# SLebailly/Ignis-MasterThesis

Measured on AMD Instinct MI355X. Metric: Mrays/s (primary+secondary) at fixed spp; per-pixel L2 vs CPU ref, higher is better.
Workload: dtype f32; 1 GPU; diamond_scene.json 1000x1000, 256 spp = 32 iterations x spi 8, path tracer max_depth 64, seed 0; scene=diamond_scene.json, width=1000, height=1000, spp=256, spi=8, parallelism=single GPU

## Files before the change

### ignis-masterthesis_amd/csrc/igx_device.hip

```cpp
#include "igx.h"

#include "device_math.h"
#include "device_scene.h"
#include "igx_kernels.h"
#include "../host/bvh_build.h"
#include "../host/light_select.h"
#include "../host/lds_plan.h"
#include "../host/aov_plan.h"
#include "../host/film_tools.h"

#include <hip/hip_runtime.h>

#include <algorithm>
#include <array>
#include <chrono>
#include <map>
#include <cmath>
#include <cstring>
#include <condition_variable>
#include <deque>
#include <memory>
#include <mutex>
#include <string>
#include <thread>
// ... 32 lines not shown

constexpr int NSH = 64;
constexpr int CSTRIDE = 16;
constexpr int CROW = NSH * CSTRIDE;
constexpr int WAVES_PER_BLOCK = BLOCK / 64;
#ifndef EXTEND_TREELET
#define EXTEND_TREELET 1
#endif
#ifndef SHADOW_TREELET
#define SHADOW_TREELET 1
#endif
#ifndef IGX_CLAIM_NEXT
#define IGX_CLAIM_NEXT 1
#endif
#ifndef IGX_LIVE_GRID
#define IGX_LIVE_GRID 1
#endif
[[maybe_unused]] constexpr int GRID_QUANTUM = NSH / WAVES_PER_BLOCK;

struct PathBuf {
    float4* p0;
    float4* p1;
    float4* p2;
    float2* p3;
    int shard_cap;
    int c_base;
};
struct ShadowBuf {
    float4* s0;
    float4* s1;
    float4* s2;
    int shard_cap;
    float4* aov_nee;
};
struct HitBuf {
    float4* h;
    int* prim;
};

#ifndef IGX_AOV
#define IGX_AOV 1
#endif
struct FrameArgs {
    int width, height, spi, iter, frame, seed;
    int tile_size, tile_offset, tile_stride, tiles_x;
    int num_rays;
    const float* rays;
    int chunk_pixel0;
    int chunk_pixels;
    int chunk_iters;
    float inv_spi;
    int gen_n;
    int classify;
    int dynamic;
    int shadow_classes;
    int reverse;
    int probe_sample;
    float4* aov_di;
    float4* aov_nee;
};

__device__ __forceinline__ void slot_coords(const FrameArgs& fa, int slot, int& lp, int& sample, int& iter) {
    const int per_iter = fa.chunk_pixels * fa.spi;
    const int it = slot / per_iter;
    const int r = slot - it * per_iter;
    const int q = r / fa.spi;
    lp = fa.chunk_pixel0 + q;
    sample = r - q * fa.spi;
    iter = fa.iter + it;
}

#ifndef IGX_PIXEL_BLOCKS
#define IGX_PIXEL_BLOCKS 1
#endif
__device__ __forceinline__ void block_order(int r, int w, int& x, int& y) {
    const int pair = r / (2 * w), q = r - pair * 2 * w;
    x = (q >> 3) * 4 + (q & 3);
    y = 2 * pair + ((q >> 2) & 1);
}
template <bool BLOCKED = true>
__device__ __forceinline__ bool local_to_global(const FrameArgs& fa, int lp, int& x, int& y) {
    if (fa.num_rays > 0) { x = lp; y = 0; return lp < fa.num_rays; }
    if (fa.tile_size <= 0) {
        if (BLOCKED && IGX_PIXEL_BLOCKS && (fa.width & 3) == 0 && (fa.height & 1) == 0) block_order(lp, fa.width, x, y);
        else { y = lp / fa.width; x = lp - y * fa.width; }
        return true;
    }
    int T = fa.tile_size;
// ... 390 lines not shown
}

__device__ __forceinline__ void phase_mark(TraceStats& st, unsigned long long& last, int k) {
    __builtin_amdgcn_s_waitcnt(0);
    __builtin_amdgcn_sched_barrier(0);
    const unsigned long long now = __builtin_amdgcn_s_memtime();
    __builtin_amdgcn_sched_barrier(0);
    st.cyc[k] += now - last;
    last = now;
}
template <bool STATS, int V>
__device__ __forceinline__ bool extend_step(const FrameArgs& fa, const SceneView& sv, const TStack& ts, PathState& ps, f3& Lacc,
                                            bool& has_l, bool& has_shadow, ShadowRec& sr, TraceStats& st) {
    float tmin, tmax;
    uint32_t rflags;
    ray_extent(fa, sv, ps.depth, ps.slot, tmin, tmax, rflags);
    int hit_ent, hit_prim;
    float hu = 0, hv = 0;
    trace_path_ray<STATS, V>(sv, ps.inside, ps.o, ps.d, tmin, tmax, rflags, ts, hit_ent, hit_prim, hu, hv, st);
    if (STATS && hit_ent >= 0) st.hits++;
    return shade_step<variant_full(V)>(fa, sv, ps, hit_ent, hit_prim, tmax, hu, hv, Lacc, has_l, has_shadow, sr);
}

__device__ __forceinline__ void add_radiance(float4* L, int slot, f3 c) {
    float4 l = L[slot];
    L[slot] = make_float4(l.x + c.x, l.y + c.y, l.z + c.z, 0);
}
template <bool ON = true>
__device__ __forceinline__ void add_aov(float4* A, int slot, f3 c) {
    if (ON && IGX_AOV && A) add_radiance(A, slot, c);
}

template <int V>
__device__ __forceinline__ bool extend_step_instrumented(const FrameArgs& fa, const SceneView& sv, const TStack& ts, float4* L,
                                                      PathState& ps, bool act, int bucket, bool& has_shadow, ShadowRec& sr,
                                                      TraceStats& st, unsigned long long& t_last) {
    int hit_ent = -1, hit_prim = -1;
    float hu = 0, hv = 0, tmin = 0, tmax = 0;
    uint32_t rflags = 0;
    bool alive = false;
    phase_mark(st, t_last, 0);
    const unsigned long long wn0 = st.wnodes, ln0 = st.nodes;
    if (act) {
        ray_extent(fa, sv, ps.depth, ps.slot, tmin, tmax, rflags);
        trace_path_ray<true, V>(sv, ps.inside, ps.o, ps.d, tmin, tmax, rflags, ts, hit_ent, hit_prim, hu, hv, st);
        if (hit_ent >= 0) st.hits++;
    }
    const unsigned long long c_tr = st.cyc[1];
    phase_mark(st, t_last, 1);
    uint32_t visits = (uint32_t)(st.nodes - ln0), witers = (uint32_t)(st.wnodes - wn0);
    for (int off = 32; off > 0; off >>= 1) {
        visits += __shfl_xor(visits, off);
        witers += __shfl_xor(witers, off);
    }
    if (lane_id() == 0) {
        st.cls[bucket] += st.cyc[1] - c_tr;
        st.cls[8 + bucket] += 1;
        st.cls[12 + bucket] += witers;
        st.cls[16 + bucket] += visits;
    }
    st.bucket = bucket;
    st.t_sub = t_last;
    unsigned long long sub0 = 0;
    for (int k = 0; k < 3; ++k) sub0 += st.cls[20 + 4 * bucket + k];
    if (act) {
        f3 Lacc;
        bool has_l;
        alive = shade_step<variant_full(V), true>(fa, sv, ps, hit_ent, hit_prim, tmax, hu, hv, Lacc, has_l, has_shadow, sr, &st);
        if (has_l) {
            add_radiance(L, ps.slot, Lacc);
            add_aov<variant_full(V)>(fa.aov_di, ps.slot, Lacc);
        }
    }
    const unsigned long long c_sh = st.cyc[2];
    phase_mark(st, t_last, 2);
    if (lane_id() == 0) {
        st.cls[4 + bucket] += st.cyc[2] - c_sh;
        unsigned long long sub1 = 0;
        for (int k = 0; k < 3; ++k) sub1 += st.cls[20 + 4 * bucket + k];
        st.cls[20 + 4 * bucket + 3] += (st.cyc[2] - c_sh) - (sub1 - sub0);
    }
    return alive;
}

template <bool STATS>
__device__ __forceinline__ void flush_stats(const TraceStats& st, unsigned long long* stats, int base, bool with_hits) {
    unsigned long long a = st.nodes, b = st.leaves, c = st.tris, e = st.blas, h = st.hits, wn = st.wnodes, wl = st.wleaves;
    unsigned long long tl = st.tlas_nodes, h0 = st.hot[0], h1 = st.hot[1], h2 = st.hot[2];
    for (int off = 32; off > 0; off >>= 1) {
        a += __shfl_down(a, off);
        b += __shfl_down(b, off);
        c += __shfl_down(c, off);
        e += __shfl_down(e, off);
        h += __shfl_down(h, off);
        wn += __shfl_down(wn, off);
        wl += __shfl_down(wl, off);
        tl += __shfl_down(tl, off);
        h0 += __shfl_down(h0, off);
        h1 += __shfl_down(h1, off);
        h2 += __shfl_down(h2, off);
    }
    if (lane_id() == 0) {
        atomicAdd(&stats[base + 0], a);
        atomicAdd(&stats[base + 1], b);
        atomicAdd(&stats[base + 2], c);
        atomicAdd(&stats[base + 3], e);
// ... 83 lines not shown
        if (lane_id() < 36) st.cls[lane_id()] = 0;
    }
    const WaveWork w = wave_work<BT>();
    int s = w.s;
    auto count_of = [&](int sh_) {
        if (gen) {
            const int g = gen_shard_count(fa.gen_n, sh_);
            return ShardCount{g, g, g};
        }
        return shard_count(kc.cnt_in, sh_);
    };
    ShardCount sc = count_of(s);
    uint64_t done = 0;
    int p0 = w.k * 64;
    int claimed = -1;
    unsigned long long t_last = STATS ? __builtin_amdgcn_s_memtime() : 0;
    for (;;) {
        if (fa.dynamic) {
            const int g = take_group(kc.work, s, done, sc.n, [&](int sh_) {
                sc = count_of(sh_);
                return sc.n;
            }, claimed);
            if (g < 0) break;
            p0 = g * 64;
        } else if (p0 >= sc.n) {
            break;
        }
        if (STATS) phase_mark(st, t_last, 3);
        const int ns = sc.n;
        int* const c_out = kc.cnt_out + s * CSTRIDE;
        int* const c_sh = kc.cnt_shadow + s * CSTRIDE;
        const int q = p0 + lane_id();
        const int pos = (fa.reverse && !gen) ? ns - 1 - q : q;
        bool alive = false, has_shadow = false;
        PathState ps;
        ShadowRec sr;
        ps.depth = 0;
        if (q < ns) {
            if (gen) {
                const int i = ((pos >> 6) << 12) | (s << 6) | (pos & 63);
                ps = camera_path(fa, sv, i);
                L[i] = make_float4(0, 0, 0, 0);
                if (variant_full(V0) && IGX_AOV && fa.aov_di) fa.aov_di[i] = fa.aov_nee[i] = make_float4(0, 0, 0, 0);
            } else {
                ps = load_path(in, path_index(in, s, pos, sc));
            }
            if (!STATS && ps.depth > 0) {
                f3 Lacc;
                bool has_l;
                alive = extend_step<STATS, V>(fa, sv, ts, ps, Lacc, has_l, has_shadow, sr, st);
                if (has_l) {
                    add_radiance(L, ps.slot, Lacc);
                    add_aov<variant_full(V0)>(fa.aov_di, ps.slot, Lacc);
                }
            }
        }
        if constexpr (STATS) {
            const int pg = (fa.reverse && !gen) ? ns - 1 - p0 : p0;
            const int bucket = gen ? 0 : (pg < sc.a ? 1 : pg < sc.ab ? 2 : 3);
            alive = extend_step_instrumented<V>(fa, sv, ts, L, ps, q < ns && ps.depth > 0, bucket, has_shadow, sr, st, t_last);
        }
        int dst, sdst;
        int* const claim = (IGX_CLAIM_NEXT && fa.dynamic && !((done >> s) & 1ull)) ? kc.work + s * CSTRIDE : nullptr;
        wave_append_paths(alive, path_class(fa.classify, sv, ps), has_shadow,
                          has_shadow && shadow_class_b(fa.shadow_classes, sv, sr.o, sr.d, sr.tmax), c_out, c_sh, out.shard_cap,
                          out.c_base, sh.shard_cap, dst, sdst, claim, &claimed);
        if (!claim) claimed = -1;
        if (alive) store_path(out, s * out.shard_cap + dst, ps);
        if (has_shadow) {
            const int e = s * sh.shard_cap + sdst;
            sh.s0[e] = make_float4(sr.o.x, sr.o.y, sr.o.z, __int_as_float(ps.slot));
            sh.s1[e] = make_float4(sr.d.x, sr.d.y, sr.d.z, sr.tmax);
            sh.s2[e] = make_float4(sr.color.x, sr.color.y, sr.color.z, 0);
        }
        if (!fa.dynamic) p0 += w.K * 64;
        if (STATS) phase_mark(st, t_last, 3);
    }
    if (STATS) flush_stats<STATS>(st, kc.stats, 0, true);
}

template <int V0, bool STATS, int WAVES, bool LDS>
__global__ void __launch_bounds__(BLOCK, WAVES) k_trace(FrameArgs fa, SceneView gsv, PathBuf in, HitBuf hits,
                                                      const int* cnt, int tail_threshold, unsigned long long* stats) {
    constexpr int V = LDS ? kernel_variant(V0, true) : V0;
    __shared__ int stack_mem[LDS_STACK * BLOCK];
    extern __shared__ float4 lds_scene[];
    const TStack ts = make_tstack(stack_mem, LDS_STACK, gsv.spill);
    if (row_total(cnt) <= tail_threshold) return;
    const SceneView sv = LDS ? stage_scene_lds<BLOCK>(gsv, lds_scene) : stage_treelet<BLOCK>(gsv, lds_scene);
    TraceStats st{0, 0, 0, 0, 0, 0, 0};
    const WaveWork w = wave_work();
    const ShardCount sc = shard_count(cnt, w.s);
    const int ns = sc.n;
    for (int pos = w.k * 64 + lane_id(); pos < ns; pos += w.K * 64) {
        const int i = path_index(in, w.s, pos, sc);
        float4 p0 = in.p0[i], p1 = in.p1[i];
        int depth = (int)(__float_as_uint(p1.w) >> 24);
        int hit_ent = -1, hit_prim = -1;
        float hu = 0, hv = 0, tmax = 0;
        if (depth > 0) {
            float tmin;
            uint32_t rflags;
            ray_extent(fa, sv, depth, (int)(__float_as_uint(p0.w) & SLOT_MASK), tmin, tmax, rflags);
            trace_ray<false, STATS, V>(sv, f3of(p0), f3of(p1), tmin, tmax, rflags, ts, hit_ent, hit_prim, hu, hv, st);
            if (STATS && hit_ent >= 0) st.hits++;
        }
// ... 198 lines not shown
                if (cont) ++bounces;
            }
            tracing = cont;
            had_shadow = has_shadow;
            const float ox = __shfl(sr.o.x, partner), oy = __shfl(sr.o.y, partner), oz = __shfl(sr.o.z, partner);
            const float dx = __shfl(sr.d.x, partner), dy = __shfl(sr.d.y, partner), dz = __shfl(sr.d.z, partner);
            const float tm = __shfl(sr.tmax, partner);
            const bool ph = __shfl(has_shadow, partner) != 0;
            if (!path_lane) {
                sh_trace = ph;
                so = mk(ox, oy, oz);
                sd = mk(dx, dy, dz);
                stmax = tm;
            }
            start = true;
        }
    }
    for (int off = 32; off > 0; off >>= 1) {
        bounces += __shfl_down(bounces, off);
        shadows += __shfl_down(shadows, off);
    }
    if (lane_id() == 0 && (bounces | shadows)) {
        atomicAdd(&tail_counts[0], bounces);
        atomicAdd(&tail_counts[1], shadows);
    }
    if (STATS) {
        flush_stats<STATS>(st, stats, 0, true);
        flush_stats<STATS>(sst, stats, 4, false);
    }
}

template <bool STATS, int V>
__device__ __forceinline__ bool shadow_walk(const SceneView& sv, const TStack& ts, float4 s0, float4 s1, float4 col, float4 l,
                                            float4* L, float4* aov_nee, TraceStats& st) {
    float tmax = s1.w;
    int e, p;
    float u, v;
    const bool occl = trace_ray<true, STATS, V>(sv, f3of(s0), f3of(s1), 0.001f, tmax, RAY_SHADOW, ts, e, p, u, v, st);
    if (!occl) {
        const int slot = __float_as_int(s0.w);
        L[slot] = make_float4(l.x + col.x, l.y + col.y, l.z + col.z, 0);
        add_aov(aov_nee, slot, f3of(col));
    }
    return occl;
}

template <int V0, bool STATS, bool LDS>
__global__ void __launch_bounds__(BLOCK) k_shadow(SceneView gsv, ShadowBuf sh, float4* L, const int* cnt,
                                                  unsigned long long* stats, int* work) {
    constexpr int V = LDS ? kernel_variant(V0, true) : (SHADOW_TREELET ? kernel_variant(V0, false) : V0);
    __shared__ int stack_mem[LDS_STACK * BLOCK];
    extern __shared__ float4 lds_scene[];
    const TStack ts = make_tstack(stack_mem, LDS_STACK, gsv.spill);
    if (row_total(cnt) == 0) return;
    const SceneView sv = LDS ? stage_scene_lds<BLOCK>(gsv, lds_scene) : stage_treelet<BLOCK>(gsv, lds_scene);
    TraceStats st{0, 0, 0, 0, 0, 0, 0};
    unsigned long long cls_acc[2][6] = {};
    const WaveWork w = wave_work();
    const int lane = lane_id();
    int s = w.s;
    ShardCount sc = shard_count(cnt, s);
    unsigned long long c0 = 0;
    uint32_t wn0 = 0, ln0 = 0;
    auto stats_begin = [&]() {
        if constexpr (STATS) {
            c0 = __builtin_amdgcn_s_memtime();
            wn0 = st.wnodes;
            ln0 = st.nodes;
        }
    };
    auto stats_end = [&](int p0, bool act, bool occl) {
        if constexpr (STATS) {
            __builtin_amdgcn_s_waitcnt(0);
            const unsigned long long c1 = __builtin_amdgcn_s_memtime();
            uint32_t visits = st.nodes - ln0, witers = st.wnodes - wn0, occ = occl ? 1 : 0, nr = act ? 1 : 0;
            for (int off = 32; off > 0; off >>= 1) {
                visits += __shfl_xor(visits, off);
                witers += __shfl_xor(witers, off);
                occ += __shfl_xor(occ, off);
                nr += __shfl_xor(nr, off);
            }
            const int cls = p0 < sc.a ? 0 : 1;
            if (lane == 0) {
                cls_acc[cls][0] += 1;
                cls_acc[cls][1] += witers;
                cls_acc[cls][2] += visits;
                cls_acc[cls][3] += c1 - c0;
                cls_acc[cls][4] += occ;
                cls_acc[cls][5] += nr;
            }
        }
    };
    {
        uint64_t done = 0;
        for (int p0 = w.k * 64;; p0 += w.K * 64) {
            if (work) {
                p0 = take_group(work, s, done, sc.n, [&](int sh_) {
                    sc = shard_count(cnt, sh_);
                    return sc.n;
                });
                if (p0 < 0) break;
                p0 *= 64;
            } else if (p0 >= sc.n) {
                break;
            }
            const int pos = p0 + lane;
            stats_begin();
            bool occl = false;
            if (pos < sc.n) {
                const int i = stream_index(s, pos, sc.a, sh.shard_cap);
                occl = shadow_walk<STATS, V>(sv, ts, sh.s0[i], sh.s1[i], sh.s2[i], L[__float_as_int(sh.s0[i].w)], L, sh.aov_nee, st);
            }
            stats_end(p0, pos < sc.n, occl);
        }
    }
    if constexpr (STATS) {
        if (lane == 0)
            for (int c = 0; c < 2; ++c)
                for (int k = 0; k < 6; ++k)
                    if (cls_acc[c][k]) atomicAdd(&stats[k < 5 ? 40 + 2 * k + c : 70 + c], cls_acc[c][k]);
    }
    if (STATS) flush_stats<STATS>(st, stats, 4, false);
}

#ifndef REFILL_WAVES
#define REFILL_WAVES 6
#endif
#ifndef REFILL_WAVES_Q4
#define REFILL_WAVES_Q4 6
#endif
#ifndef SHADOW_IFIF_WAVES
#define SHADOW_IFIF_WAVES 7
#endif
#ifndef REFILL_WAVES_LDS
#define REFILL_WAVES_LDS 4
#endif
template <bool CLASSES>
struct GroupSeq {
    const int* cnt;
    int* work;
    int shard_cap;
    WaveWork w;
    int s;
    uint64_t done;
    bool exhausted;
    int j0;
    int gs[2], gg[2], ga[2], gn[2];

    __device__ __forceinline__ ShardCount count_of(int sh) const {
        if constexpr (CLASSES) return shard_count(cnt, sh);
        const int n = uniform_load(cnt + sh * CSTRIDE);
        return ShardCount{n, n, n};
    }
    __device__ __forceinline__ void init(const int* cnt_, int* work_, int cap, const WaveWork& w_) {
        cnt = cnt_;
        work = work_;
        shard_cap = cap;
        w = w_;
        s = w.s;
        done = 0;
        exhausted = false;
        j0 = 0;
        gg[0] = gg[1] = -1;
    }
    __device__ __forceinline__ bool fill(int k) {
        if (exhausted) return false;
        ShardCount sc = count_of(s);
        int g;
        if (work) {
            g = take_group(work, s, done, sc.n, [&](int sh_) {
// ... 4 lines not shown
            g = w.k + (j0 + k) * w.K;
            if (g * 64 >= sc.n) g = -1;
        }
        if (g < 0) {
            exhausted = true;
            return false;
        }
        gs[k] = s;
        gg[k] = g;
        ga[k] = sc.a;
        gn[k] = sc.n;
        return true;
    }
    __device__ __forceinline__ bool reserve(int cursor, int m) {
        if (cursor >= (j0 + 1) * 64) {
            gs[0] = gs[1];
            gg[0] = gg[1];
            ga[0] = ga[1];
            gn[0] = gn[1];
            gg[1] = -1;
            ++j0;
        }
        if (gg[0] < 0 && !fill(0)) return false;
        if (cursor + m > (j0 + 1) * 64 && gg[1] < 0) fill(1);
        return true;
    }
    __device__ __forceinline__ bool at(int c, int& i) const {
        const int k = (c >> 6) - j0;
        const int g = k ? gg[1] : gg[0];
        if (g < 0) return false;
        const int pos = g * 64 + (c & 63);
        if (pos >= (k ? gn[1] : gn[0])) return false;
        const int sh = k ? gs[1] : gs[0];
        i = CLASSES ? stream_index(sh, pos, k ? ga[1] : ga[0], shard_cap) : sh * shard_cap + pos;
        return true;
    }
};

template <int V0, bool STATS, bool LDS>
__global__ void __launch_bounds__(BLOCK, LDS ? REFILL_WAVES_LDS : (variant_q4(V0) ? REFILL_WAVES_Q4 : REFILL_WAVES)) k_trace_refill(FrameArgs fa, SceneView gsv, PathBuf in, HitBuf hits,
                                                                     const int* cnt, int tail_threshold,
                                                                     unsigned long long* stats, int refill_min, int* work) {
    constexpr int V = LDS ? kernel_variant(V0, true) : V0;
    __shared__ int stack_mem[LDS_STACK * BLOCK];
    extern __shared__ float4 lds_scene[];
    const TStack ts = make_tstack(stack_mem, LDS_STACK, gsv.spill);
    if (row_total(cnt) <= tail_threshold) return;
    const SceneView sv = LDS ? stage_scene_lds<BLOCK>(gsv, lds_scene) : stage_treelet<BLOCK>(gsv, lds_scene);
    TraceStats st{0, 0, 0, 0, 0, 0, 0};
    GroupSeq<true> seq;
    seq.init(cnt, work, in.shard_cap, wave_work());
    refill_loop<false, STATS, V>(
        sv, ts, seq, refill_min,
        [&](int i, Trav& t) -> bool {
            const float4 p0 = in.p0[i], p1 = in.p1[i];
            const int depth = (int)(__float_as_uint(p1.w) >> 24);
            if (depth == 0) {
                hits.h[i] = make_float4(0, 0, 0, __int_as_float(-1));
                hits.prim[i] = -1;
                return false;
            }
            float tmin, tmax;
            uint32_t rflags;
            ray_extent(fa, sv, depth, (int)(__float_as_uint(p0.w) & SLOT_MASK), tmin, tmax, rflags);
            trav_init(sv, t, f3of(p0), f3of(p1), tmin, tmax, rflags, ts);
            return true;
        },
        [&](int i, const Trav& t) {
            if (STATS && t.hit_ent >= 0) st.hits++;
            hits.h[i] = make_float4(t.tmax, t.hu, t.hv, __int_as_float(t.hit_ent));
            hits.prim[i] = t.hit_prim;
        },
        st);
    if (STATS) flush_stats<STATS>(st, stats, 0, true);
}

template <int V0, bool STATS, bool LDS>
__global__ void __launch_bounds__(BLOCK, LDS ? REFILL_WAVES_LDS : (variant_ifif(V0) ? SHADOW_IFIF_WAVES : REFILL_WAVES)) k_shadow_refill(SceneView gsv, ShadowBuf sh, float4* L, const int* cnt,
                                                                      unsigned long long* stats, int refill_min, int* work) {
    constexpr int V = LDS ? kernel_variant(V0, true) : ((SHADOW_TREELET && !variant_ifif(V0)) ? kernel_variant(V0, false) : V0);
    __shared__ int stack_mem[LDS_STACK * BLOCK];
    extern __shared__ float4 lds_scene[];
    const TStack ts = make_tstack(stack_mem, LDS_STACK, gsv.spill);
    if (row_total(cnt) == 0) return;
    const SceneView sv = LDS ? stage_scene_lds<BLOCK>(gsv, lds_scene) : stage_treelet<BLOCK>(gsv, lds_scene);
    TraceStats st{0, 0, 0, 0, 0, 0, 0};
    GroupSeq<true> seq;
    seq.init(cnt, work, sh.shard_cap, wave_work());
    refill_loop<true, STATS, V>(
        sv, ts, seq, refill_min,
        [&](int i, Trav& t) -> bool {
            const float4 s0 = sh.s0[i], s1 = sh.s1[i];
            trav_init(sv, t, f3of(s0), f3of(s1), 0.001f, s1.w, RAY_SHADOW, ts);
            return true;
        },
        [&](int i, const Trav& t) {
            if (t.found) return;
            const int slot = __float_as_int(sh.s0[i].w);
            const f3 col = f3of(sh.s2[i]);
            add_radiance(L, slot, col);
            add_aov(sh.aov_nee, slot, col);
        },
        st);
    if (STATS) flush_stats<STATS>(st, stats, 4, false);
}

#if IGX_PART == 0
constexpr int RES_G = 8;
__global__ void __launch_bounds__(64 * RES_G) k_resolve(FrameArgs fa, const float4* L, float* fb, int fb_width) {
    __shared__ float part[RES_G][3][64];
    const int lane = threadIdx.x & 63, w = threadIdx.x >> 6;
    const int p = blockIdx.x * 64 + lane;
    int x = 0, y = 0;
    const bool in = p < fa.chunk_pixels && local_to_global(fa, fa.chunk_pixel0 + p, x, y);
    const size_t o = 3 * ((size_t)y * fb_width + x);
    float fr = 0, fg = 0, fbb = 0;
    if (w == 0 && in) {
        fr = fb[o + 0];
        fg = fb[o + 1];
        fbb = fb[o + 2];
    }
    for (int it0 = 0; it0 < fa.chunk_iters; it0 += RES_G) {
        const int it = it0 + w;
        if (in && it < fa.chunk_iters) {
            const float4* Li = L + ((size_t)it * fa.chunk_pixels + p) * fa.spi;
            float r = 0, g = 0, b = 0;
            if (fa.probe_sample) {
                const float4 l = Li[fa.probe_sample - 1];
                r = l.x * fa.inv_spi;
                g = l.y * fa.inv_spi;
                b = l.z * fa.inv_spi;
            } else {
#pragma unroll 8
                for (int s = 0; s < fa.spi; ++s) {
// ... 211 lines not shown
    std::string last_error;
    int num_cus = 256;
    size_t mem_total = 0;
    bool timing = false;
    bool instrument = false;
    int64_t capacity_opt = 0;
    int64_t slot_budget_mb = 0;
    int stream_slots = 2;
    int concurrent_opt = 1;
    int concurrent_start_pct = 10;
    int tail_pairs_opt = -1;
    int64_t treelet_opt = -1;
    bool tree_dirty = true;
    int tree_ext = 0, tree_shadow = 0;
    int64_t tail_opt = -1;
    int64_t tail_last_opt = -1;
    bool fuse_generate = true;
    int split_opt = -1;
    int refill_opt = -1;
    int shadow_ifif_opt = -1;
    int64_t lds_scene_max = 48 * 1024;
    size_t lds_scene_bytes = 0;
    int lds_shading_opt = -1;
    int64_t lds_shading_max = 48 * 1024;
    size_t lds_shading_bytes = 0;
    int ext_block = BLOCK;
    size_t lds_shading_tab[LDS_TAB_COUNT] = {};
    size_t lds_per_block = 64 * 1024;
    size_t table_bytes = 0;
    size_t shading_bytes = 0;
    int leaf_size = 4;
    int classify_opt = 4;
    int shadow_classes_opt = 1;
    int dynamic_opt = DYN_EXTEND | DYN_REFILL_TRACE | DYN_REFILL_SHADOW;
    int group_order_opt = -1;
    int face_normals_opt = 1;
    int face_shade_opt = 1;
    float sah_node_cost = 1.0f;
    int bvh_bins = 32;
    int bvh_bins_tlas = 32;
    bool spatial_splits = false;
    bool rebuild_bvh = false;
    bool has_scene = false;
    std::vector<void*> scene_allocs;
    SceneView sv{};
    igx_camera cam_desc{};
    int variant = 0;
    int bvh_width = 2;
    bool quantized = false;
    int quantize_opt = -1;
    int nf4 = 4;
    int bvh_width_opt = 0;
    bool full_shading = false;
    bool full_shading_opt = false;
    bool enclosing_opt = true;
    int scene_depth = 0;
    int* spill_main = nullptr;
    int* spill_tail = nullptr;
    int* spill_shadow = nullptr;
    int* spill_main2 = nullptr;
    hipStream_t shadow_stream = nullptr;
    int overlap_shadow_opt = 1;
    Slot slots[2];
    int next_slot = 0;
    unsigned long long* dstats = nullptr;
    unsigned long long* tail_counts = nullptr;
// ... 141 lines not shown
        s.ev_pool.push_back(e);
    }
    return s.ev_pool[s.ev_next++];
}

int grid_for(igx_device* dev, long long items, int blocks_per_cu, int block = BLOCK) {
    const long long q = NSH / (block / 64);
    long long need = (items + block - 1) / block;
    long long cap = (long long)dev->num_cus * std::min(blocks_per_cu, MAX_BLOCKS_PER_CU * BLOCK / block);
    long long g = std::min((need + q - 1) / q * q, std::max(q, cap / q * q));
    return (int)std::max(q, g);
}

#endif

constexpr size_t SPLIT_TABLE_BYTES = 64u << 20;
#ifndef GROUP_ORDER_AUTO
#define GROUP_ORDER_AUTO 0
#endif
inline bool use_tail_pairs(const igx_device* dev) {
    return dev->lds_scene_bytes == 0 && (dev->tail_pairs_opt < 0 ? true : dev->tail_pairs_opt != 0);
}
inline size_t tree_bytes(const igx_device* dev, int nodes) { return (size_t)nodes * dev->nf4 * 16; }
inline int refill_min(const igx_device* dev) { return dev->refill_opt >= 0 ? dev->refill_opt : 16; }
inline bool use_refill(const igx_device* dev) {
    return refill_min(dev) > 0 && (dev->lds_scene_bytes == 0 || dev->refill_opt > 0);
}
inline bool use_split(const igx_device* dev) {
    return dev->split_opt >= 0 ? dev->split_opt != 0 : (dev->lds_scene_bytes == 0 && dev->table_bytes > SPLIT_TABLE_BYTES);
}
inline bool use_shadow_ifif(const igx_device* dev) {
    return dev->shadow_ifif_opt >= 0 ? dev->shadow_ifif_opt != 0 : use_split(dev);
}

#define IGX_DISPATCH_VARIANT(v, MACRO)        \
    do {                                      \
        switch ((v) & (3 | VARIANT_Q4)) {     \
        case 0: MACRO(0); break;              \
        case 1: MACRO(1); break;              \
        case 2: MACRO(2); break;              \
        case 3: MACRO(3); break;              \
        case 2 | VARIANT_Q4: MACRO(130); break; \
        default: MACRO(131); break;           \
        }                                     \
    } while (0)
#define IGX_DISPATCH_VARIANT8(v, MACRO)       \
    do {                                      \
        switch ((v) & (7 | VARIANT_Q4)) {     \
        case 0: MACRO(0); break;              \
        case 1: MACRO(1); break;              \
        case 2: MACRO(2); break;              \
        case 3: MACRO(3); break;              \
        case 4: MACRO(4); break;              \
        case 5: MACRO(5); break;              \
        case 6: MACRO(6); break;              \
        case 7: MACRO(7); break;              \
        case 2 | VARIANT_Q4: MACRO(130); break; \
        case 3 | VARIANT_Q4: MACRO(131); break; \
        case 6 | VARIANT_Q4: MACRO(134); break; \
        default: MACRO(135); break;           \
        }                                     \
    } while (0)

template <bool STATS>
void launch_extend_wide(igx_device* dev, Slot& s, int grid, const FrameArgs& fa, const PathBuf& in, const PathBuf& out,
                        const KernelCounters& kc, int tail) {
// ... 568 lines not shown
        if (value < 0) return fail(dev, IGX_ERR_INVALID_ARGUMENT, "slot_budget_mb must be >= 0 (0 = auto)");
        dev->slot_budget_mb = value;
    }
    else if (k == "concurrent_chunks") dev->concurrent_opt = value != 0 ? 1 : 0;
    else if (k == "async_render") dev->async_opt = value != 0 ? 1 : 0;
    else if (k == "denoise_aovs") {
        if (value < INFO_OFF || value > INFO_EVERY)
            return fail(dev, IGX_ERR_INVALID_ARGUMENT, "denoise_aovs must be 0 (off), 1 (first iteration) or 2 (every iteration)");
        dev->info_mode = (int)value;
    }
    else if (k == "denoise_follow_specular") dev->info_follow_specular = value != 0;
    else if (k == "denoise_max_depth") {
        if (value < 0) return fail(dev, IGX_ERR_INVALID_ARGUMENT, "denoise_max_depth must be >= 0");
        dev->info_max_depth = (int)std::min<int64_t>(value, 1 << 20);
    }
    else if (k == "probe_sample") dev->probe_sample_opt = std::max<int64_t>(0, value);
    else if (k == "fail_chunk") dev->fail_chunk_opt = std::max<int64_t>(0, value);
    else if (k == "face_shade") dev->face_shade_opt = value != 0 ? 1 : 0;
    else if (k == "host_wait_us") dev->host_wait_us = (int)std::max<int64_t>(0, std::min<int64_t>(value, 10000));
    else if (k == "concurrent_start_pct") {
        if (value < 0 || value > 100) return fail(dev, IGX_ERR_INVALID_ARGUMENT, "concurrent_start_pct must be 0..100");
        dev->concurrent_start_pct = (int)value;
    }
    else if (k == "tail_threshold") dev->tail_opt = value;
    else if (k == "tail_threshold_last") dev->tail_last_opt = value;
    else if (k == "fuse_generate") dev->fuse_generate = value != 0;
    else if (k == "split") {
        if (value < -1 || value > 1) return fail(dev, IGX_ERR_INVALID_ARGUMENT, "split must be -1 (auto), 0 or 1");
        dev->split_opt = (int)value;
    }
    else if (k == "shadow_ifif") {
        if (value < -1 || value > 1) return fail(dev, IGX_ERR_INVALID_ARGUMENT, "shadow_ifif must be -1 (auto), 0 or 1");
        dev->shadow_ifif_opt = (int)value;
    }
    else if (k == "refill") {
        if (value < -1 || value > 64) return fail(dev, IGX_ERR_INVALID_ARGUMENT, "refill must be -1 (auto) or in [0, 64]");
        dev->refill_opt = (int)value;
    }
    else if (k == "lds_scene_max") {
        dev->lds_scene_max = value;
        configure_lds(dev);
    }
    else if (k == "lds_shading") {
        if (value < -1 || value > 1) return fail(dev, IGX_ERR_INVALID_ARGUMENT, "lds_shading must be -1 (auto), 0 or 1");
        dev->lds_shading_opt = (int)value;
        configure_lds(dev);
    }
    else if (k == "lds_shading_max") {
        dev->lds_shading_max = value;
        configure_lds(dev);
    }
    else if (k == "full_shading") dev->full_shading_opt = value != 0;
    else if (k == "enclosing") dev->enclosing_opt = value != 0;
    else if (k == "bvh_width") {
        if (value != 0 && value != 2 && value != 4) return fail(dev, IGX_ERR_INVALID_ARGUMENT, "bvh_width must be 0 (auto), 2 or 4");
        dev->bvh_width_opt = (int)value;
    }
    else if (k == "spatial_splits") dev->spatial_splits = value != 0;
    else if (k == "rebuild_bvh") dev->rebuild_bvh = value != 0;
    else if (k == "dynamic") dev->dynamic_opt = (int)(value & 15);
    else if (k == "group_order") {
        if (value < -1 || value > 1) return fail(dev, IGX_ERR_INVALID_ARGUMENT, "group_order must be -1 (auto), 0 (A, B, C) or 1 (C, B, A)");
        dev->group_order_opt = (int)value;
    }
    else if (k == "face_normals") dev->face_normals_opt = value != 0;
    else if (k == "bvh_bins") {
// ... 875 lines not shown
            break;
        }
        if (!r.loop_done && r.live * 100 > (long long)dev->concurrent_start_pct * r.n) late = false;
    }
    if (nx && late) {
        const int k = dev->stream_slots == 1 ? 0 : dev->next_slot;
        Slot& S = dev->slots[k];
        bool busy = false;
        for (const SchedItem& r : items) busy = busy || (!r.fence() && r.started && r.slot == k);
        if (!busy && S.pending) {
            const hipError_t q = hipEventQuery(S.done);
            if (q == hipErrorNotReady) busy = true;
            else IGX_CC(q);
        }
        if (!busy) {
            SchedItem& r = *nx;
            const ChunkPlan& pl = *r.plan;
            if (dev->fail_chunk_opt > 0 && --dev->fail_chunk_opt == 0) {
                restore();
                return fail(dev, IGX_ERR_HIP, "injected failure (option fail_chunk)");
            }
            igx_status st;
            if ((st = harvest(dev, S)) != IGX_OK || (st = ensure_slot(dev, S, pl.slot_cap, false, pl.fa.classify >= 4, dev->aov_on)) != IGX_OK) {
                restore();
                return st;
            }
            if (dev->stream_slots == 2) dev->next_slot ^= 1;
            r.started = true;
            r.slot = k;
            r.fa = pl.fa;
            r.fa.aov_di = dev->aov_on && dev->aov_fb[0] ? S.aov_di : nullptr;
            r.fa.aov_nee = dev->aov_on && dev->aov_fb[1] ? S.aov_nee : nullptr;
            S.sh.aov_nee = r.fa.aov_nee;
            r.fa.iter = pl.iteration + r.it0;
            r.fa.chunk_iters = std::min(pl.iters_per_chunk, pl.count - r.it0);
            r.chunk_pixels = (int)std::min<long long>(pl.chunk_pixels_max, pl.local_pixels - r.px0);
            r.fa.chunk_pixel0 = (int)r.px0;
            r.fa.chunk_pixels = r.chunk_pixels;
            r.n = (long long)r.chunk_pixels * pl.spi * r.fa.chunk_iters;
            r.live = r.n;
            const long long fin_lanes = (long long)pl.fin_bpc * dev->num_cus * BLOCK / (pl.pairs ? 2 : 1);
            const int64_t topt = r.last_of_plan && dev->tail_last_opt >= 0 ? dev->tail_last_opt : dev->tail_opt;
            r.tail = topt >= 0 ? (int)std::min<int64_t>(topt, 1 << 30) : (int)std::max<long long>(32768, std::min(r.n / 64, fin_lanes));
            S.tail = r.tail;
            S.camera = valid_pixels_in_chunk(r.fa) * pl.spi * r.fa.chunk_iters;
            S.n0 = r.n;
            S.split = false;
            S.bounce_ev.clear();
            S.launched = 0;
            r.ext_grid = grid_for(dev, r.n, pl.ext_bpc, dev->ext_block);
            r.sh_grid = grid_for(dev, r.n, pl.sh_bpc);
            r.fin_grid = grid_for(dev, std::min<long long>(r.n, r.tail) * (pl.pairs ? 2 : 1), pl.fin_bpc);
            r.fuse_gen = dev->fuse_generate && r.n > r.tail;
            use_slot(r);
            IGX_CC(hipMemsetAsync(S.ctr, 0, (size_t)(2 * pl.max_bounces + 4) * CROW * sizeof(int), dev->stream));
            if (dev->dynamic_opt)
                IGX_CC(hipMemsetAsync(S.ctr + (size_t)WORK_ROW0 * CROW, 0, (size_t)4 * pl.max_bounces * CROW * sizeof(int), dev->stream));
            if (!r.fuse_gen) {
                begin_timed(S, 2, -1, dev->stream);
                hipLaunchKernelGGL(k_generate, dim3(grid_for(dev, r.n, 8)), dim3(BLOCK), 0, dev->stream, r.fa, dev->sv, S.pa, S.L, S.ctr);
                end_timed(S, dev->stream);
                IGX_CC(hipGetLastError());
            }
            restore();
            if (r.n <= r.tail) {
                r.switch_b = 0;
// ... 285 lines not shown
        igx_status dst = drain(dev);
        if (dst != IGX_OK) return dst;
        if (dev->fb) HIPCHK(hipFree(dev->fb));
        dev->fb = nullptr;
        for (float*& a : dev->aov_fb) {
            if (a) HIPCHK(hipFree(a));
            a = nullptr;
        }
        HIPCHK(hipMalloc((void**)&dev->fb, fbc * sizeof(float)));
        HIPCHK(hipMemsetAsync(dev->fb, 0, fbc * sizeof(float), dev->tail_stream));
        if (want_aov)
            for (float*& a : dev->aov_fb) {
                HIPCHK(hipMalloc((void**)&a, fbc * sizeof(float)));
                HIPCHK(hipMemsetAsync(a, 0, fbc * sizeof(float), dev->tail_stream));
            }
        dev->fb_w = width;
        dev->fb_h = height;
        dev->fb_count = fbc;
        dev->iteration_count = 0;
    }
    const DevCamera cam = make_camera(dev, width, height);
    if (!async) dev->sv.cam = cam;

    FrameArgs fa{};
    fa.width = width;
    fa.height = height;
    fa.spi = p->spi;
    fa.iter = p->iteration;
    fa.frame = p->frame;
    fa.seed = p->seed;
    fa.inv_spi = 1.0f / (float)p->spi;
    fa.classify = dev->classify_opt;
    fa.shadow_classes = dev->shadow_classes_opt;
    fa.dynamic = dev->dynamic_opt & DYN_EXTEND;
    fa.reverse = fa.dynamic ? (dev->group_order_opt < 0 ? GROUP_ORDER_AUTO : dev->group_order_opt) : 0;
    fa.probe_sample = dev->probe_sample_opt > 0 && dev->probe_sample_opt <= p->spi ? (int)dev->probe_sample_opt : 0;
    long long local_pixels;
    if (list_mode) {
        igx_status dst = drain(dev);
        if (dst != IGX_OK) return dst;
        size_t need = (size_t)p->num_rays * 8;
        if (dev->ray_list_cap < need) {
            if (dev->ray_list) HIPCHK(hipFree(dev->ray_list));
            HIPCHK(hipMalloc((void**)&dev->ray_list, need * sizeof(float)));
            dev->ray_list_cap = need;
        }
        HIPCHK(hipMemcpy(dev->ray_list, p->rays, need * sizeof(float), hipMemcpyHostToDevice));
        fa.num_rays = p->num_rays;
        fa.rays = dev->ray_list;
        local_pixels = p->num_rays;
    } else if (p->tile_size > 0) {
        fa.tile_size = p->tile_size;
        fa.tile_offset = p->tile_offset;
        fa.tile_stride = p->tile_stride;
        fa.tiles_x = (width + p->tile_size - 1) / p->tile_size;
        int tiles_y = (height + p->tile_size - 1) / p->tile_size;
        int tiles = fa.tiles_x * tiles_y;
        int mine = tiles > p->tile_offset ? (tiles - p->tile_offset + p->tile_stride - 1) / p->tile_stride : 0;
        local_pixels = (long long)mine * p->tile_size * p->tile_size;
    } else {
        local_pixels = (long long)width * height;
    }
    if (const int64_t passes = info_passes_in(dev->info_mode, p->iteration, count); passes > 0 && dev->info_fb[0]) {
        for (uint64_t& c : dev->info_count) c += (uint64_t)passes;
        if (local_pixels > 0) {
            auto pass = std::make_shared<InfoPass>();
// ... 76 lines not shown
        plan->max_bounces = max_bounces;
        plan->ext_bpc = ext_bpc;
        plan->sh_bpc = sh_bpc;
        plan->fin_bpc = fin_bpc;
        plan->pairs = pairs;
        dev->iteration_count += count;
        dev->stats.iterations += count;
        if (async) {
            AsyncRender::Job job;
            job.plan = std::move(plan);
            submit_async(dev, std::move(job));
        } else {
            ChunkScheduler sched;
            sched.add(plan);
            igx_status st = run_scheduler(dev, sched);
            if (st != IGX_OK) return st;
        }
        dev->stats.ms_render += std::chrono::duration<double, std::milli>(std::chrono::steady_clock::now() - t_start).count();
        return IGX_OK;
    }

    for (int it0 = 0; it0 < count; it0 += iters_per_chunk)
    for (long long px0 = 0; px0 < local_pixels; px0 += chunk_pixels_max) {
        fa.iter = p->iteration + it0;
        fa.chunk_iters = std::min(iters_per_chunk, count - it0);
        Slot& S = dev->slots[dev->stream_slots == 1 ? 0 : dev->next_slot];
        dev->next_slot ^= 1;
        igx_status st = harvest(dev, S);
        if (st != IGX_OK) return st;
        if ((st = ensure_slot(dev, S, slot_cap, split, fa.classify >= 4, dev->aov_on && !list_mode)) != IGX_OK) return st;
        fa.aov_di = dev->aov_on && dev->aov_fb[0] && !list_mode ? S.aov_di : nullptr;
        fa.aov_nee = dev->aov_on && dev->aov_fb[1] && !list_mode ? S.aov_nee : nullptr;
        S.sh.aov_nee = fa.aov_nee;

        auto begin_timed = [&](int kind, int bounce, hipStream_t strm) {
            if (!dev->timing) return;
            TimedLaunch t{slot_event(S), slot_event(S), kind, bounce};
            (void)hipEventRecord(t.a, strm);
            S.timed.push_back(t);
        };
        auto end_timed = [&](hipStream_t strm) {
            if (!dev->timing) return;
            (void)hipEventRecord(S.timed.back().b, strm);
        };

        int chunk_pixels = (int)std::min<long long>(chunk_pixels_max, local_pixels - px0);
        fa.chunk_pixel0 = (int)px0;
        fa.chunk_pixels = chunk_pixels;
        long long n = (long long)chunk_pixels * p->spi * fa.chunk_iters;
        const long long fin_lanes = (long long)fin_bpc * dev->num_cus * BLOCK / (pairs ? 2 : 1);
        const bool last_chunk = it0 + iters_per_chunk >= count && px0 + chunk_pixels_max >= local_pixels;
        const int64_t topt = last_chunk && dev->tail_last_opt >= 0 ? dev->tail_last_opt : dev->tail_opt;
        int tail = topt >= 0 ? (int)std::min<int64_t>(topt, 1 << 30)
                                      : (int)std::max<long long>(32768, std::min(n / 64, fin_lanes));
        S.tail = tail;
        S.camera = valid_pixels_in_chunk(fa) * p->spi * fa.chunk_iters;
        int* cnt = S.ctr;
        auto row = [&](int r) { return cnt + (size_t)r * CROW; };
        HIPCHK(hipMemsetAsync(S.ctr, 0, (size_t)(2 * max_bounces + 4) * CROW * sizeof(int), dev->stream));
        if (dev->dynamic_opt)
            HIPCHK(hipMemsetAsync(S.ctr + (size_t)WORK_ROW0 * CROW, 0, (size_t)4 * max_bounces * CROW * sizeof(int), dev->stream));
        const bool fuse_gen = dev->fuse_generate && !split && n > tail;
        if (!fuse_gen) {
            begin_timed(2, -1, dev->stream);
            hipLaunchKernelGGL(k_generate, dim3(grid_for(dev, n, 8)), dim3(BLOCK), 0, dev->stream, fa, dev->sv, S.pa, S.L, cnt);
            end_timed(dev->stream);
// ... 498 lines not shown
```

Measured before the change: 14150 Mrays/s.

## Add optimistic shadow contribution with undo record for class-A shadow rays

For shadow rays in class A, the extend kernel now adds the NEE contribution to the radiance buffer right away. It stores the pre-add radiance in the shadow record in place of the light colour. The shadow kernels then restore that saved value only when the ray turns out to be occluded, so unoccluded rays skip a read-modify-write of L. The radiance update is also merged into one load and store per path after the wave append, and the camera-path clear of L is folded into it. The feature is auto-enabled when shadow classes are active and the scene has enclosures, but not with split mode or AOVs. It relies on each slot having only one pending shadow ray per bounce, which keeps the undo correct.

Result: faster. 14690 Mrays/s, median of 6 (+3.8%).

```diff
diff --git a/ignis-masterthesis_amd/csrc/igx_device.hip b/ignis-masterthesis_amd/csrc/igx_device.hip
--- a/ignis-masterthesis_amd/csrc/igx_device.hip
+++ b/ignis-masterthesis_amd/csrc/igx_device.hip
@@ -88,6 +88,7 @@
     float4* s2;
     int shard_cap;
     float4* aov_nee;
+    int optimistic;
 };
 struct HitBuf {
     float4* h;
@@ -110,6 +111,7 @@
     int classify;
     int dynamic;
     int shadow_classes;
+    int shadow_optimistic;
     int reverse;
     int probe_sample;
     float4* aov_di;
@@ -566,9 +568,10 @@
 }
 
 template <int V>
-__device__ __forceinline__ bool extend_step_instrumented(const FrameArgs& fa, const SceneView& sv, const TStack& ts, float4* L,
-                                                      PathState& ps, bool act, int bucket, bool& has_shadow, ShadowRec& sr,
-                                                      TraceStats& st, unsigned long long& t_last) {
+__device__ __forceinline__ bool extend_step_instrumented(const FrameArgs& fa, const SceneView& sv, const TStack& ts,
+                                                      PathState& ps, bool act, int bucket, f3& Lacc, bool& has_l,
+                                                      bool& has_shadow, ShadowRec& sr, TraceStats& st,
+                                                      unsigned long long& t_last) {
     int hit_ent = -1, hit_prim = -1;
     float hu = 0, hv = 0, tmin = 0, tmax = 0;
     uint32_t rflags = 0;
@@ -597,15 +600,7 @@
     st.t_sub = t_last;
     unsigned long long sub0 = 0;
     for (int k = 0; k < 3; ++k) sub0 += st.cls[20 + 4 * bucket + k];
-    if (act) {
-        f3 Lacc;
-        bool has_l;
-        alive = shade_step<variant_full(V), true>(fa, sv, ps, hit_ent, hit_prim, tmax, hu, hv, Lacc, has_l, has_shadow, sr, &st);
-        if (has_l) {
-            add_radiance(L, ps.slot, Lacc);
-            add_aov<variant_full(V)>(fa.aov_di, ps.slot, Lacc);
-        }
-    }
+    if (act) alive = shade_step<variant_full(V), true>(fa, sv, ps, hit_ent, hit_prim, tmax, hu, hv, Lacc, has_l, has_shadow, sr, &st);
     const unsigned long long c_sh = st.cyc[2];
     phase_mark(st, t_last, 2);
     if (lane_id() == 0) {
@@ -755,46 +750,55 @@
         int* const c_sh = kc.cnt_shadow + s * CSTRIDE;
         const int q = p0 + lane_id();
         const int pos = (fa.reverse && !gen) ? ns - 1 - q : q;
-        bool alive = false, has_shadow = false;
+        bool alive = false, has_shadow = false, has_l = false;
         PathState ps;
         ShadowRec sr;
+        f3 Lacc = mk(0, 0, 0);
         ps.depth = 0;
         if (q < ns) {
             if (gen) {
                 const int i = ((pos >> 6) << 12) | (s << 6) | (pos & 63);
                 ps = camera_path(fa, sv, i);
-                L[i] = make_float4(0, 0, 0, 0);
                 if (variant_full(V0) && IGX_AOV && fa.aov_di) fa.aov_di[i] = fa.aov_nee[i] = make_float4(0, 0, 0, 0);
             } else {
                 ps = load_path(in, path_index(in, s, pos, sc));
             }
-            if (!STATS && ps.depth > 0) {
-                f3 Lacc;
-                bool has_l;
-                alive = extend_step<STATS, V>(fa, sv, ts, ps, Lacc, has_l, has_shadow, sr, st);
-                if (has_l) {
-                    add_radiance(L, ps.slot, Lacc);
-                    add_aov<variant_full(V0)>(fa.aov_di, ps.slot, Lacc);
-                }
-            }
+            if (!STATS && ps.depth > 0) alive = extend_step<STATS, V>(fa, sv, ts, ps, Lacc, has_l, has_shadow, sr, st);
         }
         if constexpr (STATS) {
             const int pg = (fa.reverse && !gen) ? ns - 1 - p0 : p0;
             const int bucket = gen ? 0 : (pg < sc.a ? 1 : pg < sc.ab ? 2 : 3);
-            alive = extend_step_instrumented<V>(fa, sv, ts, L, ps, q < ns && ps.depth > 0, bucket, has_shadow, sr, st, t_last);
-        }
+            alive = extend_step_instrumented<V>(fa, sv, ts, ps, q < ns && ps.depth > 0, bucket, Lacc, has_l, has_shadow, sr, st, t_last);
+        }
+        const bool sh_b = has_shadow && shadow_class_b(fa.shadow_classes, sv, sr.o, sr.d, sr.tmax);
+        const bool opt_add = fa.shadow_optimistic && has_shadow && !sh_b;
+        const bool upd = gen ? q < ns : (has_l || opt_add);
+        float4 l = make_float4(0, 0, 0, 0);
+        if (!gen && upd) l = L[ps.slot];
         int dst, sdst;
         int* const claim = (IGX_CLAIM_NEXT && fa.dynamic && !((done >> s) & 1ull)) ? kc.work + s * CSTRIDE : nullptr;
-        wave_append_paths(alive, path_class(fa.classify, sv, ps), has_shadow,
-                          has_shadow && shadow_class_b(fa.shadow_classes, sv, sr.o, sr.d, sr.tmax), c_out, c_sh, out.shard_cap,
+        wave_append_paths(alive, path_class(fa.classify, sv, ps), has_shadow, sh_b, c_out, c_sh, out.shard_cap,
                           out.c_base, sh.shard_cap, dst, sdst, claim, &claimed);
         if (!claim) claimed = -1;
         if (alive) store_path(out, s * out.shard_cap + dst, ps);
+        f3 rec = sr.color;
+        if (upd) {
+            f3 v = f3of(l);
+            if (has_l) {
+                v = mk(v.x + Lacc.x, v.y + Lacc.y, v.z + Lacc.z);
+                add_aov<variant_full(V0)>(fa.aov_di, ps.slot, Lacc);
+            }
+            if (opt_add) {
+                rec = v;
+                v = mk(v.x + sr.color.x, v.y + sr.color.y, v.z + sr.color.z);
+            }
+            L[ps.slot] = make_float4(v.x, v.y, v.z, 0);
+        }
         if (has_shadow) {
             const int e = s * sh.shard_cap + sdst;
             sh.s0[e] = make_float4(sr.o.x, sr.o.y, sr.o.z, __int_as_float(ps.slot));
             sh.s1[e] = make_float4(sr.d.x, sr.d.y, sr.d.z, sr.tmax);
-            sh.s2[e] = make_float4(sr.color.x, sr.color.y, sr.color.z, 0);
+            sh.s2[e] = make_float4(rec.x, rec.y, rec.z, 0);
         }
         if (!fa.dynamic) p0 += w.K * 64;
         if (STATS) phase_mark(st, t_last, 3);
@@ -1059,16 +1063,28 @@
 
 template <bool STATS, int V>
 __device__ __forceinline__ bool shadow_walk(const SceneView& sv, const TStack& ts, float4 s0, float4 s1, float4 col, float4 l,
-                                            float4* L, float4* aov_nee, TraceStats& st) {
+                                            bool undo, float4* L, float4* aov_nee, TraceStats& st) {
     float tmax = s1.w;
     int e, p;
     float u, v;
     const bool occl = trace_ray<true, STATS, V>(sv, f3of(s0), f3of(s1), 0.001f, tmax, RAY_SHADOW, ts, e, p, u, v, st);
-    if (!occl) {
-        const int slot = __float_as_int(s0.w);
+    const int slot = __float_as_int(s0.w);
+    if (undo) {
+        if (occl) L[slot] = make_float4(col.x, col.y, col.z, 0);
+    } else if (!occl) {
         L[slot] = make_float4(l.x + col.x, l.y + col.y, l.z + col.z, 0);
         add_aov(aov_nee, slot, f3of(col));
     }
+    return occl;
+}
+template <bool STATS, int V>
+__device__ __forceinline__ bool shadow_walk_undo(const SceneView& sv, const TStack& ts, float4 s0, float4 s1, const float4* undo,
+                                                 float4* L, TraceStats& st) {
+    float tmax = s1.w;
+    int e, p;
+    float u, v;
+    const bool occl = trace_ray<true, STATS, V>(sv, f3of(s0), f3of(s1), 0.001f, tmax, RAY_SHADOW, ts, e, p, u, v, st);
+    if (occl) L[__float_as_int(s0.w)] = *undo;
     return occl;
 }
 
@@ -1134,9 +1150,15 @@
             const int pos = p0 + lane;
             stats_begin();
             bool occl = false;
-            if (pos < sc.n) {
+            if (sh.optimistic && p0 + 63 < sc.a) {
+                const int i = s * sh.shard_cap + pos;
+                occl = shadow_walk_undo<STATS, V>(sv, ts, sh.s0[i], sh.s1[i], sh.s2 + i, L, st);
+            } else if (pos < sc.n) {
                 const int i = stream_index(s, pos, sc.a, sh.shard_cap);
-                occl = shadow_walk<STATS, V>(sv, ts, sh.s0[i], sh.s1[i], sh.s2[i], L[__float_as_int(sh.s0[i].w)], L, sh.aov_nee, st);
+                const bool undo = sh.optimistic && pos < sc.a;
+                const float4 s0 = sh.s0[i];
+                const float4 l = undo ? make_float4(0, 0, 0, 0) : L[__float_as_int(s0.w)];
+                occl = shadow_walk<STATS, V>(sv, ts, s0, sh.s1[i], sh.s2[i], l, undo, L, sh.aov_nee, st);
             }
             stats_end(p0, pos < sc.n, occl);
         }
@@ -1162,7 +1184,8 @@
 #ifndef REFILL_WAVES_LDS
 #define REFILL_WAVES_LDS 4
 #endif
-template <bool CLASSES>
+constexpr int CLASS_A_TAG = (int)0x80000000u;
+template <bool CLASSES, bool TAG_A = false>
 struct GroupSeq {
     const int* cnt;
     int* work;
@@ -1233,7 +1256,9 @@
         const int pos = g * 64 + (c & 63);
         if (pos >= (k ? gn[1] : gn[0])) return false;
         const int sh = k ? gs[1] : gs[0];
-        i = CLASSES ? stream_index(sh, pos, k ? ga[1] : ga[0], shard_cap) : sh * shard_cap + pos;
+        const int a = k ? ga[1] : ga[0];
+        i = CLASSES ? stream_index(sh, pos, a, shard_cap) : sh * shard_cap + pos;
+        if (TAG_A && pos < a) i |= CLASS_A_TAG;
         return true;
     }
 };
@@ -1286,21 +1311,28 @@
     if (row_total(cnt) == 0) return;
     const SceneView sv = LDS ? stage_scene_lds<BLOCK>(gsv, lds_scene) : stage_treelet<BLOCK>(gsv, lds_scene);
     TraceStats st{0, 0, 0, 0, 0, 0, 0};
-    GroupSeq<true> seq;
+    GroupSeq<true, true> seq;
     seq.init(cnt, work, sh.shard_cap, wave_work());
     refill_loop<true, STATS, V>(
         sv, ts, seq, refill_min,
-        [&](int i, Trav& t) -> bool {
+        [&](int it, Trav& t) -> bool {
+            const int i = it & ~CLASS_A_TAG;
             const float4 s0 = sh.s0[i], s1 = sh.s1[i];
             trav_init(sv, t, f3of(s0), f3of(s1), 0.001f, s1.w, RAY_SHADOW, ts);
             return true;
         },
-        [&](int i, const Trav& t) {
-            if (t.found) return;
+        [&](int it, const Trav& t) {
+            const bool undo = sh.optimistic && it < 0;
+            if (t.found != undo) return;
+            const int i = it & ~CLASS_A_TAG;
             const int slot = __float_as_int(sh.s0[i].w);
-            const f3 col = f3of(sh.s2[i]);
-            add_radiance(L, slot, col);
-            add_aov(sh.aov_nee, slot, col);
+            const float4 rec = sh.s2[i];
+            if (undo) {
+                L[slot] = rec;
+                return;
+            }
+            add_radiance(L, slot, f3of(rec));
+            add_aov(sh.aov_nee, slot, f3of(rec));
         },
         st);
     if (STATS) flush_stats<STATS>(st, stats, 4, false);
@@ -1578,6 +1610,7 @@
     int leaf_size = 4;
     int classify_opt = 4;
     int shadow_classes_opt = 1;
+    int shadow_optimistic_opt = -1;
     int dynamic_opt = DYN_EXTEND | DYN_REFILL_TRACE | DYN_REFILL_SHADOW;
     int group_order_opt = -1;
     int face_normals_opt = 1;
@@ -1785,6 +1818,10 @@
 inline bool use_shadow_ifif(const igx_device* dev) {
     return dev->shadow_ifif_opt >= 0 ? dev->shadow_ifif_opt != 0 : use_split(dev);
 }
+inline bool use_shadow_optimistic(const igx_device* dev, bool split, bool aovs) {
+    if (dev->shadow_optimistic_opt == 0 || split || aovs) return false;
+    return dev->shadow_optimistic_opt > 0 || (dev->shadow_classes_opt && dev->sv.num_enc > 0);
+}
 
 #define IGX_DISPATCH_VARIANT(v, MACRO)        \
     do {                                      \
@@ -2419,6 +2456,10 @@
     else if (k == "shadow_ifif") {
         if (value < -1 || value > 1) return fail(dev, IGX_ERR_INVALID_ARGUMENT, "shadow_ifif must be -1 (auto), 0 or 1");
         dev->shadow_ifif_opt = (int)value;
+    }
+    else if (k == "shadow_optimistic") {
+        if (value < -1 || value > 1) return fail(dev, IGX_ERR_INVALID_ARGUMENT, "shadow_optimistic must be -1 (auto), 0 or 1");
+        dev->shadow_optimistic_opt = (int)value;
     }
     else if (k == "refill") {
         if (value < -1 || value > 64) return fail(dev, IGX_ERR_INVALID_ARGUMENT, "refill must be -1 (auto) or in [0, 64]");
@@ -3360,6 +3401,7 @@
             r.fa.aov_di = dev->aov_on && dev->aov_fb[0] ? S.aov_di : nullptr;
             r.fa.aov_nee = dev->aov_on && dev->aov_fb[1] ? S.aov_nee : nullptr;
             S.sh.aov_nee = r.fa.aov_nee;
+            S.sh.optimistic = r.fa.shadow_optimistic;
             r.fa.iter = pl.iteration + r.it0;
             r.fa.chunk_iters = std::min(pl.iters_per_chunk, pl.count - r.it0);
             r.chunk_pixels = (int)std::min<long long>(pl.chunk_pixels_max, pl.local_pixels - r.px0);
@@ -3711,6 +3753,7 @@
     fa.inv_spi = 1.0f / (float)p->spi;
     fa.classify = dev->classify_opt;
     fa.shadow_classes = dev->shadow_classes_opt;
+    fa.shadow_optimistic = use_shadow_optimistic(dev, split, dev->aov_on && !list_mode);
     fa.dynamic = dev->dynamic_opt & DYN_EXTEND;
     fa.reverse = fa.dynamic ? (dev->group_order_opt < 0 ? GROUP_ORDER_AUTO : dev->group_order_opt) : 0;
     fa.probe_sample = dev->probe_sample_opt > 0 && dev->probe_sample_opt <= p->spi ? (int)dev->probe_sample_opt : 0;
@@ -3853,6 +3896,7 @@
         fa.aov_di = dev->aov_on && dev->aov_fb[0] && !list_mode ? S.aov_di : nullptr;
         fa.aov_nee = dev->aov_on && dev->aov_fb[1] && !list_mode ? S.aov_nee : nullptr;
         S.sh.aov_nee = fa.aov_nee;
+        S.sh.optimistic = fa.shadow_optimistic;
 
         auto begin_timed = [&](int kind, int bounce, hipStream_t strm) {
             if (!dev->timing) return;
```
